# nglaze00/SCoNe_GCN

Hardware: NVIDIA B200
Metric: SCoNe train trajectories/sec (higher is better)
Workload: dtype f32

## Files before the change

### include/scone_b200.h

```cpp
#ifndef SCONE_B200_H
#define SCONE_B200_H

#include <stdint.h>

#ifdef __cplusplus
extern "C" {
#endif

#define SCONE_B200_VERSION 100
#define SCONE_MAX_DEGREE 128

typedef struct scone_complex scone_complex;
typedef struct scone_model scone_model;

enum { SCONE_MODEL_SCONE = 0, SCONE_MODEL_EBLI = 1, SCONE_MODEL_BUNCH = 2 };
enum { SCONE_ACT_TANH = 0, SCONE_ACT_LEAKY_RELU = 1, SCONE_ACT_RELU = 2 };

int scone_version(void);
const char* scone_last_error(void);

int scone_complex_create(int32_t n_nodes, int32_t n_edges, int32_t n_tris,
                         const int32_t* edge_nodes , const int8_t* edge_signs ,
                         const int32_t* tri_edges , const int8_t* tri_signs ,
                         int32_t model, scone_complex** out);
// ... 67 lines not shown
                              const float* flow_val, const int32_t* last_nodes, const int32_t* n_nbrs,
                              const int32_t* target_idx, const float* mask, int32_t* out_host , void* stream);
int scone_model_eval_host(scone_model* m, int32_t B, const int32_t* traj_ptr, const int32_t* flow_edge, const float* flow_val,
                          const int32_t* last_nodes, const int32_t* n_nbrs, const int32_t* target_idx, const float* mask,
                          int32_t* choice_out, int32_t* acc_out, float* nll_out, void* stream);
int scone_model_two_target_host(scone_model* m, int32_t B, const int32_t* true_idx, const int32_t* rand_idx, int32_t* out ,
                                void* stream);
int scone_model_read_grads(scone_model* m, float* out_host, void* stream);
int scone_model_read_grads_async(scone_model* m, float* out_pinned, void* stream);

int scone_model_adam_step(scone_model* m, int32_t step, float lr, float weight_decay, void* stream);

typedef struct scone_dp scone_dp;
int scone_dp_create(int32_t rank, int32_t world, int64_t n_floats, scone_dp** out);
int32_t scone_dp_handle_bytes(void);
int scone_dp_get_handle(scone_dp* dp, void* handle_out);
int scone_dp_open(scone_dp* dp, const void* handles_rank_major);
int scone_model_dp_adam_step(scone_model* m, scone_dp* dp, int32_t step, float lr, float wd, void* stream);
int scone_dp_status(scone_dp* dp, void* stream);
void scone_dp_destroy(scone_dp* dp);
int scone_model_plan_host(scone_model* m, int32_t B, const int32_t* traj_ptr, const int32_t* flow_edge, const float* flow_val,
                          const int32_t* last_nodes, void* stream);
int scone_model_plan_dev(scone_model* m, int32_t B, const int32_t* traj_ptr_dev, const int32_t* flow_edge_dev, const float* flow_val_dev,
                         const int32_t* last_nodes_dev, void* stream);
int scone_model_loss_grad_planned_host(scone_model* m, int32_t n, const int32_t* rows, const int32_t* target_idx, const float* mask,
                                       int32_t zero_first, void* stream);
int scone_model_loss_grad_planned_dev(scone_model* m, int32_t n, const int32_t* rows_dev, const int32_t* target_idx_dev, const float* mask_dev,
                                      int32_t zero_first, void* stream);
int scone_model_forward_planned_host(scone_model* m, int32_t n, const int32_t* rows, float* logprobs_out , void* stream);
int scone_model_check_overflow(scone_model* m, void* stream);
int scone_model_set_weights_keep_state(scone_model* m, const float* weights_host, void* stream);
int scone_model_fused_info(const scone_model* m, int32_t* out );
int scone_model_fused_read(scone_model* m, int32_t t, int32_t* hdr_out , uint32_t off, int32_t words, uint32_t* arena_out);
int scone_model_read_rows_done(scone_model* m, int64_t* out );

typedef struct scone_csr scone_csr;
typedef struct scone_bunch scone_bunch;
int scone_csr_create(int32_t rows, int32_t cols, const int32_t* rowptr , const int32_t* col, const float* val,
                     scone_csr** out);
int scone_csr_destroy(scone_csr* S);
int scone_bunch_create(const scone_csr* const* S7, int32_t n_nodes, int32_t n_edges, int32_t n_tris, int32_t max_degree,
                       const int32_t* nbrhoods , int32_t n_hidden, const int32_t* hidden,
                       int32_t micro_batch, scone_bunch** out);
int scone_bunch_destroy(scone_bunch* m);
int64_t scone_bunch_num_params(const scone_bunch* m);
float* scone_bunch_grads_dev(scone_bunch* m);
int scone_bunch_set_weights(scone_bunch* m, const float* weights_host, int32_t reset_adam);
int scone_bunch_get_weights(const scone_bunch* m, float* weights_host);
int scone_bunch_forward_host(scone_bunch* m, int32_t B, const int32_t* traj_ptr, const int32_t* flow_edge, const float* flow_val,
                             const int32_t* last_nodes, float* logprobs_out , void* stream);
int scone_bunch_loss_grad_host(scone_bunch* m, int32_t B, const int32_t* traj_ptr, const int32_t* flow_edge, const float* flow_val,
                               const int32_t* last_nodes, const int32_t* target_idx, const float* mask, int32_t zero_first,
                               void* stream);
int scone_bunch_read_grads(scone_bunch* m, float* out_host, void* stream);
int scone_bunch_adam_step(scone_bunch* m, int32_t step, float lr, float weight_decay, void* stream);

int scone_set_zero_fill(int32_t on);
int scone_get_zero_fill(void);

int scone_set_dense_kernel(int32_t which);
int scone_umma_status(void* stream);
int scone_set_dense_chunk(int32_t tiles);
int scone_get_dense_kernel(void);

int scone_profile_enable(int32_t on);
int scone_profile_reset(void);
// ... 10 lines not shown
```

### scone_gcn_b200/_lib.py

```python
import ctypes as C
import os

_HERE = os.path.dirname(os.path.abspath(__file__))
_LIB = None


class LibraryMissing(RuntimeError):
    pass


class SconeError(RuntimeError):
    pass


def library_path():
    return os.path.join(_HERE, 'libscone_b200.so')


_i32, _i64, _f32, _vp = C.c_int32, C.c_int64, C.c_float, C.c_void_p
DEFAULT_DENSE_KERNEL = 3

SIGNATURES = {
    'scone_version': (C.c_int, []),
    'scone_last_error': (C.c_char_p, []),
# ... 42 lines not shown
    'scone_model_set_pipeline': (C.c_int, [_vp, _i32]),
    'scone_model_get_pipeline': (C.c_int, [_vp]),
    'scone_model_set_weights': (C.c_int, [_vp, _vp]),
    'scone_model_get_weights': (C.c_int, [_vp, _vp]),
    'scone_model_weights_dev': (_vp, [_vp]),
    'scone_model_grads_dev': (_vp, [_vp]),
    'scone_model_forward_host': (C.c_int, [_vp, _i32, _vp, _vp, _vp, _vp, _vp, _vp]),
    'scone_model_forward_dev': (C.c_int, [_vp, _i32, _vp, _vp, _vp, _vp, _vp, _vp]),
    'scone_model_loss_grad_dev': (C.c_int, [_vp, _i32, _vp, _vp, _vp, _vp, _vp, _vp, _i32, _vp]),
    'scone_model_loss_grad_host': (C.c_int, [_vp, _i32, _vp, _vp, _vp, _vp, _vp, _vp, _i32, _vp]),
    'scone_accuracy_dev': (C.c_int, [_i32, _i32, _vp, _vp, _vp, _vp, _vp, _vp]),
    'scone_model_accuracy_host': (C.c_int, [_vp, _i32, _vp, _vp, _vp, _vp, _vp, _vp, _vp, _vp, _vp]),
    'scone_model_read_grads': (C.c_int, [_vp, _vp, _vp]),
    'scone_model_read_grads_async': (C.c_int, [_vp, _vp, _vp]),
    'scone_model_eval_host': (C.c_int, [_vp, _i32] + [_vp] * 10 + [_vp]),
    'scone_model_two_target_host': (C.c_int, [_vp, _i32, _vp, _vp, _vp, _vp]),
    'scone_model_adam_step': (C.c_int, [_vp, _i32, _f32, _f32, _vp]),
    'scone_dp_create': (C.c_int, [_i32, _i32, _i64, C.POINTER(_vp)]),
    'scone_dp_handle_bytes': (_i32, []),
    'scone_dp_get_handle': (C.c_int, [_vp, _vp]),
    'scone_dp_open': (C.c_int, [_vp, _vp]),
    'scone_model_dp_adam_step': (C.c_int, [_vp, _vp, _i32, _f32, _f32, _vp]),
    'scone_dp_status': (C.c_int, [_vp, _vp]),
    'scone_dp_destroy': (None, [_vp]),
    'scone_model_check_overflow': (C.c_int, [_vp, _vp]),
    'scone_model_plan_host': (C.c_int, [_vp, _i32, _vp, _vp, _vp, _vp, _vp]),
    'scone_model_plan_dev': (C.c_int, [_vp, _i32, _vp, _vp, _vp, _vp, _vp]),
    'scone_model_loss_grad_planned_host': (C.c_int, [_vp, _i32, _vp, _vp, _vp, _i32, _vp]),
    'scone_model_loss_grad_planned_dev': (C.c_int, [_vp, _i32, _vp, _vp, _vp, _i32, _vp]),
    'scone_model_forward_planned_host': (C.c_int, [_vp, _i32, _vp, _vp, _vp]),
    'scone_model_set_weights_keep_state': (C.c_int, [_vp, _vp, _vp]),
    'scone_model_fused_info': (C.c_int, [_vp, _vp]),
    'scone_model_fused_read': (C.c_int, [_vp, _i32, _vp, C.c_uint32, _i32, _vp]),
    'scone_model_read_rows_done': (C.c_int, [_vp, _vp]),
}


def lib():
    global _LIB
    if _LIB is not None:
        return _LIB
    path = library_path()
    if not os.path.exists(path):
        raise LibraryMissing(
            '%s not found: build it with `python __graft_entry__.py build` (or `make`). '
            'scone_gcn_b200 has no CPU fallback.' % path)
    L = C.CDLL(path)
    for name, (res, args) in SIGNATURES.items():
        f = getattr(L, name)
        f.restype, f.argtypes = res, args
    _LIB = L
    return L


def check(rc, what=''):
    if rc != 0:
        msg = lib().scone_last_error().decode('utf-8', 'replace')
        raise SconeError('%s failed (code %d): %s' % (what or 'scone call', rc, msg))


def ptr(a):
    if a is None:
        return None
    assert a.flags['C_CONTIGUOUS']
    return a.ctypes.data_as(C.c_void_p)

# ... 9 lines not shown
```

### scone_gcn_b200/csrc/fused.cuh

```cuda
#pragma once
#include "common.cuh"

constexpr int kFusedMaxL = 3;
constexpr int kFusedHdrW = 16;
constexpr int kFusedFlagOverflow = 1;
constexpr int kFusedFlagRetry = 2;

struct PlanArgs {
    const int32_t* traj_ptr;
    const int32_t* flow_edge;
    const float* flow_val;
    const int32_t* last_nodes;
    const int32_t* rank;
    const int32_t* nbrhoods;
    const int32_t* inc_ptr;
    const int2* inc_ent;
    const int32_t* mptr;
    const int2* ment;
    int N, D, E, L;
    int HS, hshift;
    const unsigned* cone_ptr;
    const uint32_t* cone_ent;
    int LV;
    int EC;
    int M;
    const unsigned long long* node_off;
    const unsigned* tb_rowptr;
    const int2* tb_ent;
    const unsigned* pair_ptr;
    const int2* tb_pairs;
    const int* pair_off;
    int* hdr;
    uint32_t* arena;
    unsigned long long* bump;
    unsigned long long arena_words;
    int* overflow;
    int tier;
    int n_work;
    int t0;
    const int* n_in;
    const int* in_list;
    int* n_retry;
    int* retry;
};

#ifdef __CUDACC__
template <int THREADS>
__device__ inline int fused_block_scan_excl(int* a, int n, int* s_warp) {
    const int tid = threadIdx.x, lane = tid & 31, warp = tid >> 5;
    const int per = (n + THREADS - 1) / THREADS;
    const int lo = min(n, tid * per), hi = min(n, lo + per);
    int sum = 0;
    for (int i = lo; i < hi; ++i) sum += a[i];
    int inc = sum;
#pragma unroll
    for (int o = 1; o < 32; o <<= 1) {
        const int v = __shfl_up_sync(0xffffffffu, inc, o);
        if (lane >= o) inc += v;
    }
    __syncthreads();
    if (lane == 31) s_warp[warp] = inc;
    __syncthreads();
    int base = 0, total = 0;
#pragma unroll
    for (int w = 0; w < THREADS / 32; ++w) {
        const int v = s_warp[w];
        if (w < warp) base += v;
        total += v;
    }
    int run = base + inc - sum;
    for (int i = lo; i < hi; ++i) {
        const int v = a[i];
        a[i] = run;
        run += v;
    }
    if (tid == 0) a[n] = total;
    __syncthreads();
    return total;
}
#endif

struct FusedState {
    int L = 0, C = 0;
    int64_t n_params = 0;
    int bound_cone = 0, bound_list = 0;
    unsigned* d_cone_ptr = nullptr;
    uint32_t* d_cone_ent = nullptr;
    unsigned long long cone_entries = 0;
    bool tb_rows = false;
    unsigned long long* d_node_off = nullptr;
    unsigned* d_tb_rowptr = nullptr;
    int2* d_tb_ent = nullptr;
    unsigned* d_pair_ptr = nullptr;
    int2* d_tb_pairs = nullptr;
    int* d_pair_off = nullptr;
    unsigned long long tb_entries = 0, tb_bytes = 0;
    int tbM0 = 0, tbLV0 = 0, tbM1 = 0, tbLV1 = 0, tbM = 0, tbLV = 0;
    size_t tb_smem0 = 0, tb_smem1 = 0, tb_smem = 0;
    bool tb_two_tiers = false, tb_mid_tier = false;
    int quantile_cone = 0;
    int HS = 0, LV = 0, EC = 0, hshift = 0;
    int HS0 = 0, LV0 = 0, EC0 = 0, hshift0 = 0;
    bool two_tiers = false;
    int flow_room = 0;
    size_t plan_smem0 = 0;
    unsigned long long worst_words = 0;
    int* d_retry = nullptr;
    size_t plan_smem = 0, traj_smem_small = 0, traj_smem_big = 0;
    int cap_rows = 0, big_rows = 0, grid_small = 0, grid_big = 0, chunk = 0;
    size_t scratch_stride = 0;
    unsigned long long arena_words = 0;
    int* d_hdr = nullptr;
    uint32_t* d_arena = nullptr;
    unsigned long long* d_bump = nullptr;
    float* d_partial = nullptr;
    float* d_scratch = nullptr;
    int* d_stats = nullptr;
    unsigned long long* d_rows_done = nullptr;
    uint32_t* d_sort = nullptr;
    void* d_sort_tmp = nullptr;
    size_t sort_tmp_bytes = 0;
    int sort_cap = 0;
    int* d_set_hdr = nullptr;
    uint32_t* d_set_arena = nullptr;
    unsigned long long* d_set_bump = nullptr;
    unsigned long long set_arena_words = 0;
    int set_cap = 0, set_n = 0;
};

int scone_table_build(const scone_complex* cx, FusedState* f, int L, bool* ok);
int scone_table_plan_launch(const FusedState* f, PlanArgs p, int b, int num_sms, cudaStream_t st, int phase = 2);
void scone_table_destroy(FusedState* f);
// ... 22 lines not shown
```

### scone_gcn_b200/csrc/scone_fused.cu

```cuda
#include <algorithm>
#include <cstdlib>
#include <cub/device/device_radix_sort.cuh>
#include "common.cuh"
#include "fused.cuh"

namespace {

#include "slab_common.cuh"

constexpr int kTrajThreads = 256;
constexpr int kFuMaxD = SCONE_MAX_DEGREE;
constexpr uint32_t kNoRow = 0xFFFFu;
constexpr uint32_t kFlaggedKey = 0xFFFFFFu;

template <int ACT>
__device__ __forceinline__ float fu_act(float z) {
    if (ACT == SCONE_ACT_TANH) return scone_tanh(z);
    if (ACT == SCONE_ACT_LEAKY_RELU) return z >= 0.f ? z : 0.01f * z;
    return fmaxf(z, 0.f);
}
template <int ACT>
__device__ __forceinline__ float fu_dact(float h) {
    if (ACT == SCONE_ACT_TANH) return 1.f - h * h;
    if (ACT == SCONE_ACT_LEAKY_RELU) return h >= 0.f ? 1.f : 0.01f;
// ... 1095 lines not shown
    f->cap_rows = C == 32 ? 192 : 384;
    f->big_rows = L * f->bound_list;
    f->traj_smem_small = C == 32 ? traj_smem_bytes<32>(cx->D, f->cap_rows) : traj_smem_bytes<16>(cx->D, f->cap_rows);
    f->traj_smem_big = C == 32 ? traj_smem_bytes<32>(cx->D, 0) : traj_smem_bytes<16>(cx->D, 0);
    if (f->traj_smem_small > 113 * 1024) {
        const size_t over = f->traj_smem_small - 113 * 1024;
        const int less = (int)((over + ldh * 4 - 1) / (ldh * 4));
        f->cap_rows = f->cap_rows > less + 32 ? f->cap_rows - less : 32;
        f->traj_smem_small = C == 32 ? traj_smem_bytes<32>(cx->D, f->cap_rows) : traj_smem_bytes<16>(cx->D, f->cap_rows);
    }
    f->grid_small = 2 * cx->num_sms;
    f->grid_big = f->big_rows > f->cap_rows ? 2 * cx->num_sms : 0;
    if (f->grid_big) {
        f->scratch_stride = (size_t)f->big_rows * ldh;
        SCONE_CUDA(cudaMalloc((void**)&f->d_scratch, (size_t)f->grid_big * f->scratch_stride * sizeof(float)));
    }
    SCONE_CUDA(cudaMalloc((void**)&f->d_partial, (size_t)(f->grid_small + f->grid_big) * (n_params + 2) * sizeof(float)));
    const unsigned long long bl = (unsigned long long)f->bound_list;
    unsigned long long worst = 3 * bl + 2 + (unsigned long long)(cx->D + 3) + 2ull * cx->D * cx->D + 16;
    for (int l = 2; l <= L; ++l)
        worst += 2 * (bl + 3) + 4 * bl * (unsigned long long)max_row;
    const unsigned long long budget_words = (1ull << 30) - 1024;
    const unsigned long long share_words = 16 * 1024;
    f->worst_words = worst;
    if (worst * (unsigned long long)mb <= budget_words) {
        f->chunk = mb;
        f->arena_words = worst * (unsigned long long)mb;
    } else {
        f->chunk = (int)std::min<unsigned long long>((unsigned long long)mb, std::max<unsigned long long>(1, budget_words / std::min(worst, share_words)));
        f->arena_words = std::min(budget_words, worst * (unsigned long long)f->chunk);
    }
    SCONE_CUDA(cudaMalloc((void**)&f->d_arena, f->arena_words * sizeof(uint32_t)));
    SCONE_CUDA(cudaMalloc((void**)&f->d_hdr, (size_t)f->chunk * kFusedHdrW * sizeof(int)));
    SCONE_CUDA(cudaMalloc((void**)&f->d_retry, 2 * (size_t)f->chunk * sizeof(int)));
    SCONE_CUDA(cudaMalloc((void**)&f->d_bump, 2 * sizeof(unsigned long long)));
    SCONE_CUDA(cudaMalloc((void**)&f->d_rows_done, 4 * sizeof(unsigned long long)));
    SCONE_CUDA(cudaMemset(f->d_rows_done, 0, 4 * sizeof(unsigned long long)));
    *out = f;
    return 0;
}

static int launch_plans(const scone_complex* cx, const FusedState* f, PlanArgs p, int b, cudaStream_t st) {
    if (f->tb_rows) return scone_table_plan_launch(f, p, b, cx->num_sms, st);
    p.tier = 0; p.n_work = b;
    p.HS = f->HS0; p.LV = f->LV0; p.EC = f->EC0; p.hshift = f->hshift0;
    int* retry = p.retry;
    if (!f->two_tiers) p.retry = nullptr;
    fused_plan_kernel<256><<<b, 256, f->plan_smem0, st>>>(p);
    SCONE_LAUNCHED();
    if (f->two_tiers) {
        p.tier = 1; p.HS = f->HS; p.LV = f->LV; p.EC = f->EC; p.hshift = f->hshift; p.n_in = p.n_retry; p.in_list = retry; p.retry = nullptr;
        fused_plan_kernel<1024><<<std::min(b, cx->num_sms), 1024, f->plan_smem, st>>>(p);
        SCONE_LAUNCHED();
    }
    return 0;
}

int scone_fused_begin(FusedState* f, cudaStream_t st) {
    SCONE_CUDA(cudaMemsetAsync(f->d_bump, 0, 2 * sizeof(unsigned long long), st));
    return 0;
}

static PlanArgs plan_args(const scone_complex* cx, FusedState* f, int off, const int32_t* traj_ptr, const int32_t* flow_edge,
                          const float* flow_val, const int32_t* last_nodes, int* overflow) {
    PlanArgs p{};
    p.traj_ptr = traj_ptr + off; p.flow_edge = flow_edge; p.flow_val = flow_val; p.last_nodes = last_nodes + off;
    p.rank = cx->d_rank; p.nbrhoods = cx->d_nbrhoods; p.inc_ptr = cx->d_inc_ptr; p.inc_ent = cx->d_inc_ent;
    p.mptr = cx->d_mptr; p.ment = cx->d_ment; p.cone_ptr = f->d_cone_ptr; p.cone_ent = f->d_cone_ent;
// ... 31 lines not shown
    t.hdr = f->d_hdr; t.arena = f->d_arena; t.rows = nullptr; t.W = W;
    for (int i = 0; i <= 3 * kFusedMaxL; ++i) t.w_off[i] = i <= 3 * f->L ? (int)w_off[i] : 0;
    t.L = f->L; t.b = b; t.D = cx->D; t.n_params = (int)f->n_params;
    t.logprobs = logprobs; t.target_idx = target_idx; t.mask = mask;
    t.partial = f->d_partial; t.scratch = f->d_scratch; t.scratch_stride = f->scratch_stride;
    t.cap_rows = f->cap_rows; t.big_rows = f->big_rows;
    t.rows_done = count_rows ? f->d_rows_done : nullptr;
    return run_traj(f, act, t, grad, st);
}

int scone_fused_run(const scone_complex* cx, FusedState* f, int act, int b, const int32_t* traj_ptr, const int32_t* flow_edge,
                    const float* flow_val, const int32_t* last_nodes, const float* W, const int64_t* w_off, float* logprobs,
                    const int32_t* target_idx, const float* mask, float* grad, int* overflow, bool count_rows, cudaStream_t st) {
    if (b <= 0) return 0;
    SCONE_REQUIRE(b <= f->chunk, "scone_fused_run: chunk of %d trajectories exceeds the planned %d", b, f->chunk);
    int rc = scone_fused_begin(f, st);
    if (!rc) rc = scone_fused_plan_part(cx, f, 0, b, traj_ptr, flow_edge, flow_val, last_nodes, overflow, st);
    if (!rc) rc = scone_fused_compute(cx, f, act, b, W, w_off, logprobs, target_idx, mask, grad, count_rows, st);
    return rc;
}

int scone_fused_plan_set(const scone_complex* cx, FusedState* f, int B, const int32_t* traj_ptr, const int32_t* flow_edge,
                         const float* flow_val, const int32_t* last_nodes, int* overflow, cudaStream_t st) {
    if (B > f->set_cap) {
        cudaFree(f->d_set_hdr);
        cudaFree(f->d_set_arena);
        f->d_set_hdr = nullptr;
        f->d_set_arena = nullptr;
        f->set_cap = 0;
        const unsigned long long budget_words = (1ull << 30) - 1024;
        f->set_arena_words = std::min(budget_words, f->worst_words * (unsigned long long)B);
        SCONE_CUDA(cudaMalloc((void**)&f->d_set_hdr, (size_t)B * kFusedHdrW * sizeof(int)));
        SCONE_CUDA(cudaMalloc((void**)&f->d_set_arena, f->set_arena_words * sizeof(uint32_t)));
        if (!f->d_set_bump) SCONE_CUDA(cudaMalloc((void**)&f->d_set_bump, 2 * sizeof(unsigned long long)));
        f->set_cap = B;
    }
    f->set_n = 0;
    SCONE_CUDA(cudaMemsetAsync(f->d_set_bump, 0, 2 * sizeof(unsigned long long), st));
    PlanArgs p{};
    p.flow_edge = flow_edge; p.flow_val = flow_val;
    p.rank = cx->d_rank; p.nbrhoods = cx->d_nbrhoods; p.inc_ptr = cx->d_inc_ptr; p.inc_ent = cx->d_inc_ent;
    p.mptr = cx->d_mptr; p.ment = cx->d_ment; p.cone_ptr = f->d_cone_ptr; p.cone_ent = f->d_cone_ent;
    p.N = cx->N; p.D = cx->D; p.E = cx->E; p.L = f->L;
    p.arena = f->d_set_arena; p.bump = f->d_set_bump; p.arena_words = f->set_arena_words; p.overflow = overflow;
    p.n_retry = reinterpret_cast<int*>(f->d_set_bump + 1); p.retry = f->d_retry;
    ScopedProf prof(SCONE_K_CONE, st);
    for (int off = 0; off < B; off += f->chunk) {
        const int b = std::min(f->chunk, B - off);
        SCONE_CUDA(cudaMemsetAsync(f->d_set_bump + 1, 0, sizeof(unsigned long long), st));
        p.traj_ptr = traj_ptr + off; p.last_nodes = last_nodes + off; p.hdr = f->d_set_hdr + (size_t)off * kFusedHdrW;
        const int rc = launch_plans(cx, f, p, b, st);
        if (rc) return rc;
    }
    f->set_n = B;
    return 0;
}

int scone_fused_run_planned(const scone_complex* cx, FusedState* f, int act, int n, const int32_t* rows_dev, const float* W, const int64_t* w_off,
                            float* logprobs, const int32_t* target_idx, const float* mask, float* grad, bool count_rows, cudaStream_t st) {
    if (n <= 0) return 0;
    SCONE_REQUIRE(f->set_n > 0, "scone_fused_run_planned: no planned set (call scone_model_plan_* first)");
    SCONE_REQUIRE(rows_dev != nullptr || n <= f->set_n, "scone_fused_run_planned: %d trajectories requested, the planned set holds %d", n, f->set_n);
    TrajArgs t;
    t.hdr = f->d_set_hdr; t.arena = f->d_set_arena; t.rows = rows_dev; t.W = W;
    for (int i = 0; i <= 3 * kFusedMaxL; ++i) t.w_off[i] = i <= 3 * f->L ? (int)w_off[i] : 0;
    t.L = f->L; t.b = n; t.D = cx->D; t.n_params = (int)f->n_params;
    t.logprobs = logprobs; t.target_idx = target_idx; t.mask = mask;
// ... 20 lines not shown
```

### scone_gcn_b200/csrc/scone_model.cu

```cuda
#include <algorithm>
#include <cstring>
#include "common.cuh"
#include "fused.cuh"

struct scone_model {
    const scone_complex* cx = nullptr;
    int32_t L = 0, mb = 0, act = 0, cmax = 0;
    std::vector<int32_t> hidden;
    std::vector<int64_t> w_off;
    int64_t n_params = 0;
    float *d_w = nullptr, *d_m = nullptr, *d_v = nullptr, *d_grad = nullptr;
    float* d_X = nullptr;
    std::vector<float*> d_H;
    std::vector<float*> d_G;
    std::vector<uint8_t*> d_occH;
    std::vector<uint8_t*> d_occG;
    cudaStream_t side = nullptr;
    cudaStream_t compute = nullptr;
    cudaEvent_t ev_fork = nullptr, ev_join = nullptr;
    cudaEvent_t ev_begin = nullptr;
    cudaStream_t copy = nullptr;
    cudaEvent_t ev_copy0 = nullptr, ev_part[8] = {nullptr, nullptr, nullptr, nullptr, nullptr, nullptr, nullptr, nullptr};
    cudaEvent_t ev_plan_done = nullptr;
    long long staging_epoch = 0, plan_done_epoch = -1;
// ... 1051 lines not shown
    cudaStream_t s = as_stream(st);
    if (m->d_overflow) SCONE_CUDA(cudaMemcpyAsync(&overflow, m->d_overflow, sizeof(int), cudaMemcpyDeviceToHost, s));
    SCONE_CUDA(cudaStreamSynchronize(s));
    if (overflow) {
        cudaMemset(m->d_overflow, 0, sizeof(int));
        m->cone_clean = false;
        scone_set_error("scone_model: a micro-batch exceeded a row-list capacity (%d rows per compact tensor, %d rows of the backward's A "
                        "buffer, 2048 cone edges per trajectory and layer); results since the last check are incomplete and Adam steps were "
                        "skipped — use a smaller micro-batch or another pipeline", m->row_cap, m->a_cap);
        return 4;
    }
    return 0;
}

extern "C" int scone_model_set_weights_keep_state(scone_model* m, const float* w, void* st) {
    SCONE_REQUIRE(m && w, "scone_model_set_weights_keep_state: NULL argument");
    SCONE_CUDA(cudaMemcpyAsync(m->d_w, w, m->n_params * sizeof(float), cudaMemcpyHostToDevice, as_stream(st)));
    return 0;
}

extern "C" int scone_model_fused_info(const scone_model* m, int32_t* out ) {
    SCONE_REQUIRE(m && out, "scone_model_fused_info: NULL argument");
    for (int i = 0; i < 16; ++i) out[i] = 0;
    if (!m->fused) return 0;
    const FusedState* f = m->fused;
    out[0] = 1; out[1] = f->bound_cone; out[2] = f->bound_list; out[3] = f->HS; out[4] = f->chunk; out[5] = f->cap_rows;
    out[6] = (int32_t)(f->plan_smem / 1024); out[7] = (int32_t)(f->traj_smem_small / 1024);
    out[8] = f->HS0; out[9] = f->LV0; out[10] = (int32_t)(f->plan_smem0 / 1024); out[11] = f->two_tiers ? 1 : 0;
    out[12] = f->tb_rows ? (int32_t)std::max<unsigned long long>(1, f->tb_bytes >> 20) : 0; out[13] = (int32_t)(f->arena_words >> 20);
    out[14] = (int32_t)std::min<unsigned long long>(f->cone_entries >> 10, 0x7fffffffull); out[15] = scone_fused_last_retries(m->fused);
    return 0;
}

extern "C" int scone_model_fused_read(scone_model* m, int32_t t, int32_t* hdr_out, uint32_t off, int32_t words, uint32_t* arena_out) {
    SCONE_REQUIRE(m && m->fused, "scone_model_fused_read: the model has no fused pipeline");
    SCONE_REQUIRE(t >= 0 && t < m->fused->chunk && (uint64_t)off + (uint64_t)(words > 0 ? words : 0) <= m->fused->arena_words,
                  "scone_model_fused_read: out of range");
    return scone_fused_read(m->fused, t, hdr_out, off, words, arena_out);
}

extern "C" int scone_model_read_rows_done(scone_model* m, int64_t* out ) {
    SCONE_REQUIRE(m && out, "scone_model_read_rows_done: NULL argument");
    out[0] = out[1] = 0;
    if (!m->fused) return 0;
    unsigned long long v[2];
    SCONE_CUDA(cudaMemcpy(v, m->fused->d_rows_done, sizeof(v), cudaMemcpyDeviceToHost));
    SCONE_CUDA(cudaMemset(m->fused->d_rows_done, 0, sizeof(v)));
    out[0] = (int64_t)v[0];
    out[1] = (int64_t)v[1];
    return 0;
}

extern "C" int scone_umma_status(void* st) { return scone_umma_check(as_stream(st)); }

extern "C" int scone_model_dp_adam_step(scone_model* m, scone_dp* dp, int32_t step, float lr, float wd, void* st) {
    SCONE_REQUIRE(m && dp && step >= 0, "scone_model_dp_adam_step: bad arguments");
    return scone_dp_allreduce_adam(dp, m->d_w, m->d_m, m->d_v, m->d_grad, m->n_params, m->d_overflow, step, lr, wd, as_stream(st));
}

extern "C" int scone_model_adam_step(scone_model* m, int32_t step, float lr, float wd, void* st) {
    SCONE_REQUIRE(m && step >= 0, "scone_model_adam_step: bad arguments");
    return scone_adam_launch(m->d_w, m->d_m, m->d_v, m->d_grad, m->n_params, step, lr, wd, st, m->d_overflow);
}
```

### scone_gcn_b200/csrc/scone_plan_table.cu

```cuda
#include <algorithm>
#include <cstdlib>
#include <vector>
#include "common.cuh"
#include "fused.cuh"

namespace {

constexpr int kTbThreads = 256;
constexpr int kTbHS = 32768;
constexpr int kTbLC = 16384;
constexpr uint32_t kEdgeMask = 0x3FFFFFFFu;
constexpr uint32_t kEmpty = 0xFFFFFFFFu;
constexpr uint32_t kNoRow = 0xFFFFu;
constexpr int kTbMaxD = SCONE_MAX_DEGREE;
constexpr int kTbBuckets = 1024;

__device__ __forceinline__ int align2(int x) { return (x + 1) & ~1; }

struct BuildArgs {
    const int32_t* nbrhoods;
    const int32_t* inc_ptr;
    const int2* inc_ent;
    const int32_t* mptr;
    const int2* ment;
    int N, D, L;
    int* stats;
    int* cnt_m;
    unsigned* cnt_e;
    int* cnt_p;
    const unsigned* cone_ptr;
    uint32_t* keys;
    int with_rows;
    const unsigned long long* node_off;
    unsigned* rowptr;
    int2* ent;
    const unsigned* pair_ptr;
    int2* pairs;
    int* pair_off;
};

__device__ __forceinline__ int find_sorted(const uint32_t* s, int m, uint32_t e) {
    int lo = 0, hi = m;
    while (lo < hi) {
        const int mid = (lo + hi) >> 1;
        if ((s[mid] & kEdgeMask) < e) lo = mid + 1;
        else hi = mid;
    }
    return lo < m && (s[lo] & kEdgeMask) == e ? lo : -1;
}

__global__ void __launch_bounds__(kTbThreads) table_build_kernel(const BuildArgs a) {
    extern __shared__ __align__(16) unsigned char sm[];
    uint32_t* hk = reinterpret_cast<uint32_t*>(sm);
    uint32_t* list = hk + kTbHS;
    __shared__ int s_ptr[kTbMaxD], s_off[kTbMaxD + 1];
    __shared__ int s_nlist, s_m, s_n1, s_ovf, s_nat[kFusedMaxL + 2], s_warp[kTbThreads / 32];
    __shared__ unsigned s_etot;
    const int tid = threadIdx.x, lane = tid & 31, ql = tid & 3;
    const unsigned qmask = 0xFu << (lane & ~3);
    const int node = blockIdx.x, D = a.D, L = a.L;
    const bool fill = a.keys != nullptr;
    for (int i = tid; i < kTbHS; i += kTbThreads) hk[i] = kEmpty;
// ... 62 lines not shown
    __syncthreads();
    int f0 = 0;
    for (int lv = L - 1; lv >= 0; --lv) {
        const int f1 = s_nat[lv + 1];
        if (!s_ovf)
            for (int i = f0 + (tid >> 2); i < f1; i += kTbThreads / 4) {
                const int e = (int)list[i];
                const int p1 = a.mptr[e + 1];
                for (int q = a.mptr[e] + ql; q < p1; q += 4) add((uint32_t)a.ment[q].x, lv);
            }
        __syncthreads();
        if (tid == 0) s_nat[lv] = min(s_nlist, kTbLC);
        __syncthreads();
        f0 = f1;
    }
    const int m = s_m;
    const bool bad = s_ovf != 0 || m > cap;
    if (!fill) {
        if (!bad) {
            unsigned c = 0;
            const int n1 = s_nlist;
            for (int i = tid >> 2; i < n1; i += kTbThreads / 4) {
                const int e = (int)list[i];
                const int p1 = a.mptr[e + 1];
                for (int q = a.mptr[e] + ql; q < p1; q += 4) c += level_of((uint32_t)a.ment[q].x) == 0 ? 2u : 1u;
            }
            if (c) atomicAdd(&s_etot, c);
        }
        __syncthreads();
        if (tid == 0) {
            a.cnt_m[node] = bad ? 0 : m;
            a.cnt_e[node] = bad ? 0u : s_etot;
            a.cnt_p[node] = total_pairs;
            if (bad) a.stats[2] = 1;
            else {
                atomicMax(&a.stats[0], m);
                atomicMax(&a.stats[1], s_n1);
                atomicMax(&a.stats[3], total_pairs);
                atomicAdd(&a.stats[4 + min(kTbBuckets - 1, m / 32)], 1);
            }
        }
        return;
    }
    if (bad) {
        if (tid == 0) a.stats[2] = 1;
        return;
    }
    __syncthreads();
    uint32_t* tmp = hk;
    for (int i = tid; i < m; i += kTbThreads) tmp[i] = kout[i];
    __syncthreads();
    uint32_t* sorted = list;
    for (int k = tid; k < m; k += kTbThreads) {
        const uint32_t v = tmp[k], e = v & kEdgeMask;
        int r = 0;
        for (int q = 0; q < m; ++q) r += (tmp[q] & kEdgeMask) < e ? 1 : 0;
        sorted[r] = v;
    }
    __syncthreads();
    for (int i = tid; i < m; i += kTbThreads) kout[i] = sorted[i];
    if (a.with_rows) {
        for (int i = tid; i < total_pairs; i += kTbThreads) {
            const int j = slot_of(i);
            const int2 es = a.inc_ent[s_ptr[j] + (i - s_off[j])];
            const int li = find_sorted(sorted, m, (uint32_t)es.x);
            a.pairs[a.pair_ptr[node] + i] = make_int2((int)((li >= 0 ? (uint32_t)li : kNoRow) | ((uint32_t)j << 16)), es.y);
// ... 361 lines not shown
    {
        const uint16_t* idxL = idx + (L - 1) * M;
        int* pdst = reinterpret_cast<int*>(a.arena + off_ro);
        int2* edst = reinterpret_cast<int2*>(a.arena + off_ro + align2(D + 1));
        for (int j = tid; j <= D; j += THREADS) pdst[j] = last_ok ? a.pair_off[(size_t)last * (D + 1) + j] : 0;
        for (int i = tid; i < total_pairs; i += THREADS) {
            const int2 pr = a.tb_pairs[pp0 + i];
            const uint32_t li = (uint32_t)pr.x & 0xFFFFu;
            const uint32_t r = li != kNoRow ? (uint32_t)idxL[li] : kNoRow;
            edst[i] = make_int2((int)(r | ((uint32_t)pr.x & 0xFFFF0000u)), pr.y);
        }
    }
    if (tid == 0) {
        hdr[0] = 0;
        for (int l = 1; l <= kFusedMaxL; ++l) hdr[l] = l <= L ? n_l[l] : 0;
        hdr[4] = (int)off_l1;
        for (int l = 2; l <= kFusedMaxL; ++l) {
            hdr[5 + (l - 2)] = (int)off_f[l];
            hdr[7 + (l - 2)] = (int)off_b[l];
        }
        hdr[9] = (int)off_ro;
        hdr[10] = total_pairs;
        hdr[11] = m;
        hdr[12] = tot_f[2];
        hdr[13] = fp1 - fp0;
        hdr[14] = tot_f[3];
        hdr[15] = min(tot_b[2], 0xFFFF) | (min(tot_b[3], 0xFFFF) << 16);
    }
}

template <int THREADS>
__global__ void __launch_bounds__(THREADS) table_plan_kernel(const PlanArgs a) {
    extern __shared__ __align__(16) unsigned char sm[];
    const int n_work = a.tier == 0 ? a.n_work : *a.n_in;
    for (int w = blockIdx.x; w < n_work; w += gridDim.x) {
        table_plan_trajectory<THREADS>(a, a.tier == 0 ? a.t0 + w : a.in_list[w], sm);
        __syncthreads();
    }
}

constexpr int kTier1Threads = 512;
constexpr size_t kMaxTablePlanSmem = 220 * 1024;

}

void scone_table_destroy(FusedState* f) {
    cudaFree(f->d_cone_ptr); cudaFree(f->d_cone_ent); cudaFree(f->d_node_off); cudaFree(f->d_tb_rowptr); cudaFree(f->d_tb_ent);
    cudaFree(f->d_pair_ptr); cudaFree(f->d_tb_pairs); cudaFree(f->d_pair_off);
    f->d_cone_ptr = nullptr; f->d_cone_ent = nullptr; f->d_node_off = nullptr; f->d_tb_rowptr = nullptr; f->d_tb_ent = nullptr;
    f->d_pair_ptr = nullptr; f->d_tb_pairs = nullptr; f->d_pair_off = nullptr;
    f->tb_rows = false;
}

int scone_table_build(const scone_complex* cx, FusedState* f, int L, bool* ok) {
    *ok = false;
    const int N = cx->N, D = cx->D;
    if (D > kTbMaxD || N < 1) return 0;
    const int n_stats = 4 + kTbBuckets;
    SCONE_CUDA(cudaMalloc((void**)&f->d_stats, n_stats * sizeof(int)));
    SCONE_CUDA(cudaMemset(f->d_stats, 0, n_stats * sizeof(int)));
    const size_t smem = (size_t)kTbHS * 4 + (size_t)kTbLC * 4;
    SCONE_CUDA(cudaFuncSetAttribute(table_build_kernel, cudaFuncAttributeMaxDynamicSharedMemorySize, (int)smem));
    int* d_cnt_m = nullptr;
    unsigned* d_cnt_e = nullptr;
    int* d_cnt_p = nullptr;
    SCONE_CUDA(cudaMalloc((void**)&d_cnt_m, (size_t)N * sizeof(int)));
    SCONE_CUDA(cudaMalloc((void**)&d_cnt_e, (size_t)N * sizeof(unsigned)));
    SCONE_CUDA(cudaMalloc((void**)&d_cnt_p, (size_t)N * sizeof(int)));
    BuildArgs a{};
    a.nbrhoods = cx->d_nbrhoods; a.inc_ptr = cx->d_inc_ptr; a.inc_ent = cx->d_inc_ent; a.mptr = cx->d_mptr; a.ment = cx->d_ment;
    a.N = N; a.D = D; a.L = L; a.stats = f->d_stats;
    a.cnt_m = d_cnt_m; a.cnt_e = d_cnt_e; a.cnt_p = d_cnt_p;
    table_build_kernel<<<N, kTbThreads, smem>>>(a);
    SCONE_LAUNCHED();
    std::vector<int> st(n_stats), cm((size_t)N), cp((size_t)N);
    std::vector<unsigned> ce((size_t)N);
    SCONE_CUDA(cudaMemcpy(st.data(), f->d_stats, n_stats * sizeof(int), cudaMemcpyDeviceToHost));
    SCONE_CUDA(cudaMemcpy(cm.data(), d_cnt_m, (size_t)N * sizeof(int), cudaMemcpyDeviceToHost));
    SCONE_CUDA(cudaMemcpy(ce.data(), d_cnt_e, (size_t)N * sizeof(unsigned), cudaMemcpyDeviceToHost));
    SCONE_CUDA(cudaMemcpy(cp.data(), d_cnt_p, (size_t)N * sizeof(int), cudaMemcpyDeviceToHost));
    cudaFree(d_cnt_m); cudaFree(d_cnt_e); cudaFree(d_cnt_p);
    std::vector<unsigned> cone_ptr((size_t)N + 1), pair_ptr((size_t)N + 1);
    std::vector<unsigned long long> node_off((size_t)N + 1);
    unsigned long long tm = 0, te = 0, tp = 0;
    for (int n = 0; n < N; ++n) {
        cone_ptr[n] = (unsigned)tm; node_off[n] = te; pair_ptr[n] = (unsigned)tp;
        tm += (unsigned long long)cm[n]; te += ce[n]; tp += (unsigned long long)cp[n];
    }
    if (st[2] || tm + (unsigned long long)N + 1 >= (1ull << 32) || tp >= (1ull << 32)) return 0;
    cone_ptr[N] = (unsigned)tm; node_off[N] = te; pair_ptr[N] = (unsigned)tp;
    f->cone_entries = tm;
    int quantile999 = 0;
    f->bound_cone = st[0] > 0 ? st[0] : 1;
    f->bound_list = st[1] > 0 ? st[1] : 1;
    {
        long long acc = 0, want = ((long long)N * 99 + 99) / 100;
        int q0 = 32 * kTbBuckets;
        for (int b = 0; b < kTbBuckets; ++b) {
            acc += st[4 + b];
            if (acc >= want) {
                q0 = 32 * (b + 1);
                break;
            }
        }
        f->quantile_cone = std::min(q0, f->bound_cone);
        acc = 0;
        want = ((long long)N * 999 + 999) / 1000;
        quantile999 = f->bound_cone;
        for (int b = 0; b < kTbBuckets; ++b) {
            acc += st[4 + b];
            if (acc >= want) {
                quantile999 = std::min(32 * (b + 1), f->bound_cone);
                break;
            }
        }
    }
    const unsigned long long bytes = te * 8 + (tm + (unsigned long long)N + 1) * 4 + tp * 8 + (unsigned long long)N * (D + 1) * 4 + ((unsigned long long)N + 1) * 16;
    bool want_rows = true;
    {
        const char* v = getenv("SCONE_FUSED_TABLE");
        if (v && *v == '0') want_rows = false;
        size_t free_b = 0, total_b = 0;
        SCONE_CUDA(cudaMemGetInfo(&free_b, &total_b));
        if (bytes > free_b / 3) want_rows = false;
        f->tbM = (f->bound_cone + 63) & ~63;
        f->tbLV = (f->bound_list + 63) & ~63;
        f->tb_smem = table_plan_smem(f->tbM, f->tbLV);
        if (f->tb_smem > kMaxTablePlanSmem || f->bound_cone >= 0xFFFF || f->bound_list >= 0xFFFF) want_rows = false;
    }
    SCONE_CUDA(cudaMalloc((void**)&f->d_cone_ptr, cone_ptr.size() * sizeof(unsigned)));
    SCONE_CUDA(cudaMalloc((void**)&f->d_cone_ent, (size_t)(tm ? tm : 1) * sizeof(uint32_t)));
    SCONE_CUDA(cudaMemcpy(f->d_cone_ptr, cone_ptr.data(), cone_ptr.size() * sizeof(unsigned), cudaMemcpyHostToDevice));
    a.cnt_m = nullptr; a.cnt_e = nullptr; a.cnt_p = nullptr;
    a.cone_ptr = f->d_cone_ptr; a.keys = f->d_cone_ent; a.with_rows = want_rows ? 1 : 0;
    if (want_rows) {
        SCONE_CUDA(cudaMalloc((void**)&f->d_node_off, node_off.size() * sizeof(unsigned long long)));
        SCONE_CUDA(cudaMalloc((void**)&f->d_tb_rowptr, (size_t)(tm + N + 1) * sizeof(unsigned)));
        SCONE_CUDA(cudaMalloc((void**)&f->d_tb_ent, (size_t)(te ? te : 1) * sizeof(int2)));
        SCONE_CUDA(cudaMalloc((void**)&f->d_pair_ptr, pair_ptr.size() * sizeof(unsigned)));
        SCONE_CUDA(cudaMalloc((void**)&f->d_tb_pairs, (size_t)(tp ? tp : 1) * sizeof(int2)));
        SCONE_CUDA(cudaMalloc((void**)&f->d_pair_off, (size_t)N * (D + 1) * sizeof(int)));
        SCONE_CUDA(cudaMemcpy(f->d_node_off, node_off.data(), node_off.size() * sizeof(unsigned long long), cudaMemcpyHostToDevice));
        SCONE_CUDA(cudaMemcpy(f->d_pair_ptr, pair_ptr.data(), pair_ptr.size() * sizeof(unsigned), cudaMemcpyHostToDevice));
        a.node_off = f->d_node_off; a.rowptr = f->d_tb_rowptr; a.ent = f->d_tb_ent;
        a.pair_ptr = f->d_pair_ptr; a.pairs = f->d_tb_pairs; a.pair_off = f->d_pair_off;
    }
    table_build_kernel<<<N, kTbThreads, smem>>>(a);
    SCONE_LAUNCHED();
    SCONE_CUDA(cudaDeviceSynchronize());
    SCONE_CUDA(cudaMemcpy(st.data(), f->d_stats, 4 * sizeof(int), cudaMemcpyDeviceToHost));
    if (st[2] == 1) return 0;
    if (st[2] == 2) {
        want_rows = false;
        SCONE_CUDA(cudaMemset(f->d_stats + 2, 0, sizeof(int)));
        cudaFree(f->d_node_off); cudaFree(f->d_tb_rowptr); cudaFree(f->d_tb_ent); cudaFree(f->d_pair_ptr); cudaFree(f->d_tb_pairs); cudaFree(f->d_pair_off);
        f->d_node_off = nullptr; f->d_tb_rowptr = nullptr; f->d_tb_ent = nullptr; f->d_pair_ptr = nullptr; f->d_tb_pairs = nullptr; f->d_pair_off = nullptr;
    }
    f->tb_rows = want_rows;
    if (want_rows) {
        f->tb_entries = te;
        f->tb_bytes = bytes;
        auto env_int = [](const char* name, int dflt) {
            const char* v = getenv(name);
            return v && *v ? atoi(v) : dflt;
        };
        f->tbM0 = std::min(f->tbM, (env_int("SCONE_TABLE_M0", f->quantile_cone) + 63) & ~63);
        f->tbLV0 = std::min(f->tbLV, (env_int("SCONE_TABLE_LV0", 192) + 63) & ~63);
        f->tb_two_tiers = f->tbM0 < f->tbM || f->tbLV0 < f->tbLV;
        f->tb_smem0 = table_plan_smem(f->tbM0, f->tbLV0);
        f->tbM1 = std::min(f->tbM, (env_int("SCONE_TABLE_M1", std::max(quantile999, 2 * f->tbM0)) + 63) & ~63);
        f->tbLV1 = std::min(f->tbLV, (env_int("SCONE_TABLE_LV1", 512) + 63) & ~63);
        f->tb_smem1 = table_plan_smem(f->tbM1, f->tbLV1);
        f->tb_mid_tier = f->tb_two_tiers && (f->tbM1 > f->tbM0 || f->tbLV1 > f->tbLV0) && 2 * f->tb_smem1 <= f->tb_smem;
        SCONE_CUDA(cudaFuncSetAttribute(table_plan_kernel<64>, cudaFuncAttributeMaxDynamicSharedMemorySize, (int)kMaxTablePlanSmem));
        SCONE_CUDA(cudaFuncSetAttribute(table_plan_kernel<128>, cudaFuncAttributeMaxDynamicSharedMemorySize, (int)kMaxTablePlanSmem));
        SCONE_CUDA(cudaFuncSetAttribute(table_plan_kernel<256>, cudaFuncAttributeMaxDynamicSharedMemorySize, (int)kMaxTablePlanSmem));
        SCONE_CUDA(cudaFuncSetAttribute(table_plan_kernel<kTier1Threads>, cudaFuncAttributeMaxDynamicSharedMemorySize, (int)kMaxTablePlanSmem));
    }
    *ok = true;
    return 0;
}

int scone_table_plan_launch(const FusedState* f, PlanArgs p, int b, int num_sms, cudaStream_t st, int phase) {
    const int f_chunk = f->chunk;
    p.cone_ptr = f->d_cone_ptr; p.cone_ent = f->d_cone_ent; p.node_off = f->d_node_off; p.tb_rowptr = f->d_tb_rowptr; p.tb_ent = f->d_tb_ent;
    p.pair_ptr = f->d_pair_ptr; p.tb_pairs = f->d_tb_pairs; p.pair_off = f->d_pair_off;
    p.tier = 0; p.n_work = b;
    p.M = f->tbM0; p.LV = f->tbLV0;
    int* list0 = p.retry;
    int* list1 = p.retry + f_chunk;
    int* cnt0 = p.n_retry;
    int* cnt1 = p.n_retry + 1;
    p.retry = f->tb_two_tiers ? list0 : nullptr;
    p.n_retry = cnt0;
    if (phase != 1) {
        static const int t0 = [] { const char* v = getenv("SCONE_TABLE_T0"); return v && *v ? atoi(v) : 128; }();
        if (t0 == 64) table_plan_kernel<64><<<b, 64, f->tb_smem0, st>>>(p);
        else if (t0 == 256) table_plan_kernel<256><<<b, 256, f->tb_smem0, st>>>(p);
        else table_plan_kernel<128><<<b, 128, f->tb_smem0, st>>>(p);
        SCONE_LAUNCHED();
    }
    if (!f->tb_two_tiers || phase == 0) return 0;
    const int* n_in = cnt0;
    const int* in_list = list0;
    if (f->tb_mid_tier) {
        p.tier = 1; p.M = f->tbM1; p.LV = f->tbLV1; p.n_in = n_in; p.in_list = in_list; p.retry = list1; p.n_retry = cnt1;
        const int per_sm = std::max(1, std::min(8, (int)((size_t)220 * 1024 / (f->tb_smem1 + 1024))));
        table_plan_kernel<256><<<std::min(b, per_sm * num_sms), 256, f->tb_smem1, st>>>(p);
        SCONE_LAUNCHED();
        n_in = cnt1;
        in_list = list1;
    }
    p.tier = 2; p.M = f->tbM; p.LV = f->tbLV; p.n_in = n_in; p.in_list = in_list; p.retry = nullptr; p.n_retry = cnt0;
    const int per_sm = std::max(1, std::min(4, (int)((size_t)220 * 1024 / (f->tb_smem + 1024))));
    table_plan_kernel<512><<<std::min(b, per_sm * num_sms), 512, f->tb_smem, st>>>(p);
    SCONE_LAUNCHED();
    return 0;
}
```

Before: 7.431 million.

## Route trajectories to plan tiers up front and overlap tier kernels with PDL

Cone sizes per node are classified into tiers at table build time, and a small routing kernel sends each trajectory straight to its tier list by its last node. The heavy tier-2 kernel is launched first, and the mid and tier-0 kernels follow as programmatic dependent launches so they can overlap with it. This replaces the serial retry cascade, where every trajectory first tried tier 0 and overflowed down through the tiers. A fallback tier-2 pass runs only if a node's level count can exceed its tier limit, at the cost of an extra routing launch and more complex scheduling.

```diff
diff --git a/include/scone_b200.h b/include/scone_b200.h
--- a/include/scone_b200.h
+++ b/include/scone_b200.h
@@ -123,6 +123,7 @@
 int scone_model_set_weights_keep_state(scone_model* m, const float* weights_host, void* stream);
 int scone_model_fused_info(const scone_model* m, int32_t* out );
 int scone_model_fused_read(scone_model* m, int32_t t, int32_t* hdr_out , uint32_t off, int32_t words, uint32_t* arena_out);
+int scone_model_plan_tiers(const scone_model* m, int32_t* params , uint8_t* tiers);
 int scone_model_read_rows_done(scone_model* m, int64_t* out );
 
 typedef struct scone_csr scone_csr;
diff --git a/scone_gcn_b200/_lib.py b/scone_gcn_b200/_lib.py
--- a/scone_gcn_b200/_lib.py
+++ b/scone_gcn_b200/_lib.py
@@ -98,6 +98,7 @@
     'scone_model_set_weights_keep_state': (C.c_int, [_vp, _vp, _vp]),
     'scone_model_fused_info': (C.c_int, [_vp, _vp]),
     'scone_model_fused_read': (C.c_int, [_vp, _i32, _vp, C.c_uint32, _i32, _vp]),
+    'scone_model_plan_tiers': (C.c_int, [_vp, _vp, _vp]),
     'scone_model_read_rows_done': (C.c_int, [_vp, _vp]),
 }
 
diff --git a/scone_gcn_b200/csrc/fused.cuh b/scone_gcn_b200/csrc/fused.cuh
--- a/scone_gcn_b200/csrc/fused.cuh
+++ b/scone_gcn_b200/csrc/fused.cuh
@@ -42,6 +42,7 @@
     const int* in_list;
     int* n_retry;
     int* retry;
+    const uint8_t* node_tier;
 };
 
 #ifdef __CUDACC__
@@ -98,6 +99,9 @@
     int tbM0 = 0, tbLV0 = 0, tbM1 = 0, tbLV1 = 0, tbM = 0, tbLV = 0;
     size_t tb_smem0 = 0, tb_smem1 = 0, tb_smem = 0;
     bool tb_two_tiers = false, tb_mid_tier = false;
+    uint8_t* d_tier = nullptr;
+    int tb_tier_nodes[3] = {0, 0, 0};
+    bool tb_tier_retry = false;
     int quantile_cone = 0;
     int HS = 0, LV = 0, EC = 0, hshift = 0;
     int HS0 = 0, LV0 = 0, EC0 = 0, hshift0 = 0;
diff --git a/scone_gcn_b200/csrc/scone_fused.cu b/scone_gcn_b200/csrc/scone_fused.cu
--- a/scone_gcn_b200/csrc/scone_fused.cu
+++ b/scone_gcn_b200/csrc/scone_fused.cu
@@ -1151,8 +1151,8 @@
     }
     SCONE_CUDA(cudaMalloc((void**)&f->d_arena, f->arena_words * sizeof(uint32_t)));
     SCONE_CUDA(cudaMalloc((void**)&f->d_hdr, (size_t)f->chunk * kFusedHdrW * sizeof(int)));
-    SCONE_CUDA(cudaMalloc((void**)&f->d_retry, 2 * (size_t)f->chunk * sizeof(int)));
-    SCONE_CUDA(cudaMalloc((void**)&f->d_bump, 2 * sizeof(unsigned long long)));
+    SCONE_CUDA(cudaMalloc((void**)&f->d_retry, 3 * (size_t)f->chunk * sizeof(int)));
+    SCONE_CUDA(cudaMalloc((void**)&f->d_bump, 3 * sizeof(unsigned long long)));
     SCONE_CUDA(cudaMalloc((void**)&f->d_rows_done, 4 * sizeof(unsigned long long)));
     SCONE_CUDA(cudaMemset(f->d_rows_done, 0, 4 * sizeof(unsigned long long)));
     *out = f;
@@ -1250,7 +1250,7 @@
         f->set_arena_words = std::min(budget_words, f->worst_words * (unsigned long long)B);
         SCONE_CUDA(cudaMalloc((void**)&f->d_set_hdr, (size_t)B * kFusedHdrW * sizeof(int)));
         SCONE_CUDA(cudaMalloc((void**)&f->d_set_arena, f->set_arena_words * sizeof(uint32_t)));
-        if (!f->d_set_bump) SCONE_CUDA(cudaMalloc((void**)&f->d_set_bump, 2 * sizeof(unsigned long long)));
+        if (!f->d_set_bump) SCONE_CUDA(cudaMalloc((void**)&f->d_set_bump, 3 * sizeof(unsigned long long)));
         f->set_cap = B;
     }
     f->set_n = 0;
diff --git a/scone_gcn_b200/csrc/scone_model.cu b/scone_gcn_b200/csrc/scone_model.cu
--- a/scone_gcn_b200/csrc/scone_model.cu
+++ b/scone_gcn_b200/csrc/scone_model.cu
@@ -1107,6 +1107,17 @@
     return 0;
 }
 
+extern "C" int scone_model_plan_tiers(const scone_model* m, int32_t* params, uint8_t* tiers) {
+    SCONE_REQUIRE(m && params, "scone_model_plan_tiers: NULL argument");
+    for (int i = 0; i < 8; ++i) params[i] = 0;
+    const FusedState* f = m->fused;
+    if (!f || !f->d_tier) return 0;
+    params[0] = 1; params[1] = f->tbM0; params[2] = f->tbLV0; params[3] = f->tbM1; params[4] = f->tbLV1; params[5] = f->tbM;
+    params[6] = f->tbLV; params[7] = f->tb_mid_tier ? 1 : 0;
+    if (tiers) SCONE_CUDA(cudaMemcpy(tiers, f->d_tier, (size_t)m->cx->N, cudaMemcpyDeviceToHost));
+    return 0;
+}
+
 extern "C" int scone_model_fused_read(scone_model* m, int32_t t, int32_t* hdr_out, uint32_t off, int32_t words, uint32_t* arena_out) {
     SCONE_REQUIRE(m && m->fused, "scone_model_fused_read: the model has no fused pipeline");
     SCONE_REQUIRE(t >= 0 && t < m->fused->chunk && (uint64_t)off + (uint64_t)(words > 0 ? words : 0) <= m->fused->arena_words,
diff --git a/scone_gcn_b200/csrc/scone_plan_table.cu b/scone_gcn_b200/csrc/scone_plan_table.cu
--- a/scone_gcn_b200/csrc/scone_plan_table.cu
+++ b/scone_gcn_b200/csrc/scone_plan_table.cu
@@ -1,5 +1,6 @@
 #include <algorithm>
 #include <cstdlib>
+#include <cstring>
 #include <vector>
 #include "common.cuh"
 #include "fused.cuh"
@@ -28,6 +29,7 @@
     int* cnt_m;
     unsigned* cnt_e;
     int* cnt_p;
+    int* cnt_n1;
     const unsigned* cone_ptr;
     uint32_t* keys;
     int with_rows;
@@ -156,6 +158,7 @@
             a.cnt_m[node] = bad ? 0 : m;
             a.cnt_e[node] = bad ? 0u : s_etot;
             a.cnt_p[node] = total_pairs;
+            a.cnt_n1[node] = bad ? 0 : s_n1;
             if (bad) a.stats[2] = 1;
             else {
                 atomicMax(&a.stats[0], m);
@@ -583,11 +586,51 @@
 template <int THREADS>
 __global__ void __launch_bounds__(THREADS) table_plan_kernel(const PlanArgs a) {
     extern __shared__ __align__(16) unsigned char sm[];
+    asm volatile("griddepcontrol.launch_dependents;");
     const int n_work = a.tier == 0 ? a.n_work : *a.n_in;
     for (int w = blockIdx.x; w < n_work; w += gridDim.x) {
-        table_plan_trajectory<THREADS>(a, a.tier == 0 ? a.t0 + w : a.in_list[w], sm);
+        const int t = a.tier == 0 ? a.t0 + w : a.in_list[w];
+        if (a.node_tier != nullptr) {
+            const int last = a.last_nodes[t];
+            if (last >= 0 && last < a.N && a.node_tier[last] != 0) continue;
+        }
+        table_plan_trajectory<THREADS>(a, t, sm);
         __syncthreads();
     }
+    if (blockIdx.x == gridDim.x - 1) asm volatile("griddepcontrol.wait;" ::: "memory");
+}
+
+__global__ void table_route_kernel(const int32_t* last_nodes, int t0, int b, int N, const uint8_t* node_tier, int* list1, int* list2,
+                                   int* cnt) {
+    const int w = blockIdx.x * blockDim.x + threadIdx.x;
+    if (w >= b) return;
+    const int t = t0 + w;
+    const int last = last_nodes[t];
+    const int k = last >= 0 && last < N ? node_tier[last] : 0;
+    if (k == 1) list1[atomicAdd(&cnt[0], 1)] = t;
+    else if (k == 2) list2[atomicAdd(&cnt[1], 1)] = t;
+}
+
+int env_per_sm(const char* name) {
+    const char* v = getenv(name);
+    return v && *v ? atoi(v) : 0;
+}
+
+template <typename Kernel>
+int launch_dependent(Kernel kern, int grid, int threads, size_t smem, cudaStream_t st, const PlanArgs& p) {
+    cudaLaunchAttribute attr[1];
+    attr[0].id = cudaLaunchAttributeProgrammaticStreamSerialization;
+    attr[0].val.programmaticStreamSerializationAllowed = 1;
+    cudaLaunchConfig_t cfg = {};
+    cfg.gridDim = dim3((unsigned)grid);
+    cfg.blockDim = dim3((unsigned)threads);
+    cfg.dynamicSmemBytes = smem;
+    cfg.stream = st;
+    cfg.attrs = attr;
+    cfg.numAttrs = 1;
+    SCONE_CUDA(cudaLaunchKernelEx(&cfg, kern, p));
+    SCONE_LAUNCHED();
+    return 0;
 }
 
 constexpr int kTier1Threads = 512;
@@ -597,7 +640,8 @@
 
 void scone_table_destroy(FusedState* f) {
     cudaFree(f->d_cone_ptr); cudaFree(f->d_cone_ent); cudaFree(f->d_node_off); cudaFree(f->d_tb_rowptr); cudaFree(f->d_tb_ent);
-    cudaFree(f->d_pair_ptr); cudaFree(f->d_tb_pairs); cudaFree(f->d_pair_off);
+    cudaFree(f->d_pair_ptr); cudaFree(f->d_tb_pairs); cudaFree(f->d_pair_off); cudaFree(f->d_tier);
+    f->d_tier = nullptr;
     f->d_cone_ptr = nullptr; f->d_cone_ent = nullptr; f->d_node_off = nullptr; f->d_tb_rowptr = nullptr; f->d_tb_ent = nullptr;
     f->d_pair_ptr = nullptr; f->d_tb_pairs = nullptr; f->d_pair_off = nullptr;
     f->tb_rows = false;
@@ -615,22 +659,25 @@
     int* d_cnt_m = nullptr;
     unsigned* d_cnt_e = nullptr;
     int* d_cnt_p = nullptr;
+    int* d_cnt_n1 = nullptr;
     SCONE_CUDA(cudaMalloc((void**)&d_cnt_m, (size_t)N * sizeof(int)));
     SCONE_CUDA(cudaMalloc((void**)&d_cnt_e, (size_t)N * sizeof(unsigned)));
     SCONE_CUDA(cudaMalloc((void**)&d_cnt_p, (size_t)N * sizeof(int)));
+    SCONE_CUDA(cudaMalloc((void**)&d_cnt_n1, (size_t)N * sizeof(int)));
     BuildArgs a{};
     a.nbrhoods = cx->d_nbrhoods; a.inc_ptr = cx->d_inc_ptr; a.inc_ent = cx->d_inc_ent; a.mptr = cx->d_mptr; a.ment = cx->d_ment;
     a.N = N; a.D = D; a.L = L; a.stats = f->d_stats;
-    a.cnt_m = d_cnt_m; a.cnt_e = d_cnt_e; a.cnt_p = d_cnt_p;
+    a.cnt_m = d_cnt_m; a.cnt_e = d_cnt_e; a.cnt_p = d_cnt_p; a.cnt_n1 = d_cnt_n1;
     table_build_kernel<<<N, kTbThreads, smem>>>(a);
     SCONE_LAUNCHED();
-    std::vector<int> st(n_stats), cm((size_t)N), cp((size_t)N);
+    std::vector<int> st(n_stats), cm((size_t)N), cp((size_t)N), cn1((size_t)N);
     std::vector<unsigned> ce((size_t)N);
     SCONE_CUDA(cudaMemcpy(st.data(), f->d_stats, n_stats * sizeof(int), cudaMemcpyDeviceToHost));
     SCONE_CUDA(cudaMemcpy(cm.data(), d_cnt_m, (size_t)N * sizeof(int), cudaMemcpyDeviceToHost));
     SCONE_CUDA(cudaMemcpy(ce.data(), d_cnt_e, (size_t)N * sizeof(unsigned), cudaMemcpyDeviceToHost));
     SCONE_CUDA(cudaMemcpy(cp.data(), d_cnt_p, (size_t)N * sizeof(int), cudaMemcpyDeviceToHost));
-    cudaFree(d_cnt_m); cudaFree(d_cnt_e); cudaFree(d_cnt_p);
+    SCONE_CUDA(cudaMemcpy(cn1.data(), d_cnt_n1, (size_t)N * sizeof(int), cudaMemcpyDeviceToHost));
+    cudaFree(d_cnt_m); cudaFree(d_cnt_e); cudaFree(d_cnt_p); cudaFree(d_cnt_n1);
     std::vector<unsigned> cone_ptr((size_t)N + 1), pair_ptr((size_t)N + 1);
     std::vector<unsigned long long> node_off((size_t)N + 1);
     unsigned long long tm = 0, te = 0, tp = 0;
@@ -682,7 +729,7 @@
     SCONE_CUDA(cudaMalloc((void**)&f->d_cone_ptr, cone_ptr.size() * sizeof(unsigned)));
     SCONE_CUDA(cudaMalloc((void**)&f->d_cone_ent, (size_t)(tm ? tm : 1) * sizeof(uint32_t)));
     SCONE_CUDA(cudaMemcpy(f->d_cone_ptr, cone_ptr.data(), cone_ptr.size() * sizeof(unsigned), cudaMemcpyHostToDevice));
-    a.cnt_m = nullptr; a.cnt_e = nullptr; a.cnt_p = nullptr;
+    a.cnt_m = nullptr; a.cnt_e = nullptr; a.cnt_p = nullptr; a.cnt_n1 = nullptr;
     a.cone_ptr = f->d_cone_ptr; a.keys = f->d_cone_ent; a.with_rows = want_rows ? 1 : 0;
     if (want_rows) {
         SCONE_CUDA(cudaMalloc((void**)&f->d_node_off, node_off.size() * sizeof(unsigned long long)));
@@ -727,6 +774,17 @@
         SCONE_CUDA(cudaFuncSetAttribute(table_plan_kernel<128>, cudaFuncAttributeMaxDynamicSharedMemorySize, (int)kMaxTablePlanSmem));
         SCONE_CUDA(cudaFuncSetAttribute(table_plan_kernel<256>, cudaFuncAttributeMaxDynamicSharedMemorySize, (int)kMaxTablePlanSmem));
         SCONE_CUDA(cudaFuncSetAttribute(table_plan_kernel<kTier1Threads>, cudaFuncAttributeMaxDynamicSharedMemorySize, (int)kMaxTablePlanSmem));
+        std::vector<uint8_t> tier((size_t)N);
+        for (int n = 0; n < N; ++n) {
+            int k = 2;
+            if (cm[n] <= f->tbM0) k = 0;
+            else if (f->tb_mid_tier && cm[n] <= f->tbM1) k = 1;
+            if ((k == 0 && cn1[n] > f->tbLV0) || (k == 1 && cn1[n] > f->tbLV1)) f->tb_tier_retry = true;
+            tier[n] = (uint8_t)k;
+            ++f->tb_tier_nodes[k];
+        }
+        SCONE_CUDA(cudaMalloc((void**)&f->d_tier, (size_t)N));
+        SCONE_CUDA(cudaMemcpy(f->d_tier, tier.data(), (size_t)N, cudaMemcpyHostToDevice));
     }
     *ok = true;
     return 0;
@@ -740,15 +798,45 @@
     p.M = f->tbM0; p.LV = f->tbLV0;
     int* list0 = p.retry;
     int* list1 = p.retry + f_chunk;
+    int* list2 = p.retry + 2 * f_chunk;
     int* cnt0 = p.n_retry;
     int* cnt1 = p.n_retry + 1;
+    int* cnt_route = p.n_retry + 2;
+    static const int t0 = [] { const char* v = getenv("SCONE_TABLE_T0"); return v && *v ? atoi(v) : 128; }();
+    auto (*tier0_kernel) = t0 == 64 ? table_plan_kernel<64> : (t0 == 256 ? table_plan_kernel<256> : table_plan_kernel<128>);
+    const int tier0_threads = t0 == 64 || t0 == 256 ? t0 : 128;
+    const char* sched = getenv("SCONE_PLAN_SCHEDULE");
+    const bool routed = f->tb_two_tiers && f->d_tier != nullptr && !(sched && strcmp(sched, "serial") == 0);
+    if (routed) {
+        if (phase != 1 && b > 0) {
+            SCONE_CUDA(cudaMemsetAsync(cnt_route, 0, 2 * sizeof(int), st));
+            table_route_kernel<<<(b + 255) / 256, 256, 0, st>>>(p.last_nodes, p.t0, b, p.N, f->d_tier, list1, list2, cnt_route);
+            SCONE_LAUNCHED();
+            const int per_sm_env[2] = {env_per_sm("SCONE_PLAN_TIER1_CTAS"), env_per_sm("SCONE_PLAN_TIER2_CTAS")};
+            const int per_sm1 = per_sm_env[0] > 0 ? per_sm_env[0] : std::max(1, std::min(8, (int)((size_t)220 * 1024 / (f->tb_smem1 + 1024))));
+            const int per_sm2 = per_sm_env[1] > 0 ? per_sm_env[1] : std::max(1, std::min(4, (int)((size_t)220 * 1024 / (f->tb_smem + 1024))));
+            PlanArgs h = p;
+            h.retry = nullptr;
+            h.tier = 2; h.M = f->tbM; h.LV = f->tbLV; h.n_in = cnt_route + 1; h.in_list = list2;
+            table_plan_kernel<kTier1Threads><<<std::min(b, per_sm2 * num_sms), kTier1Threads, f->tb_smem, st>>>(h);
+            SCONE_LAUNCHED();
+            if (f->tb_mid_tier) {
+                h.tier = 1; h.M = f->tbM1; h.LV = f->tbLV1; h.n_in = cnt_route; h.in_list = list1; h.retry = list0; h.n_retry = cnt0;
+                if (launch_dependent(table_plan_kernel<256>, std::min(b, per_sm1 * num_sms), 256, f->tb_smem1, st, h)) return 1;
+            }
+            p.retry = list0; p.n_retry = cnt0; p.node_tier = f->d_tier;
+            if (launch_dependent(tier0_kernel, b, tier0_threads, f->tb_smem0, st, p)) return 1;
+        }
+        if (phase == 0 || !f->tb_tier_retry) return 0;
+        p.tier = 2; p.M = f->tbM; p.LV = f->tbLV; p.n_in = cnt0; p.in_list = list0; p.retry = nullptr; p.node_tier = nullptr;
+        table_plan_kernel<kTier1Threads><<<std::min(b, num_sms), kTier1Threads, f->tb_smem, st>>>(p);
+        SCONE_LAUNCHED();
+        return 0;
+    }
     p.retry = f->tb_two_tiers ? list0 : nullptr;
     p.n_retry = cnt0;
     if (phase != 1) {
-        static const int t0 = [] { const char* v = getenv("SCONE_TABLE_T0"); return v && *v ? atoi(v) : 128; }();
-        if (t0 == 64) table_plan_kernel<64><<<b, 64, f->tb_smem0, st>>>(p);
-        else if (t0 == 256) table_plan_kernel<256><<<b, 256, f->tb_smem0, st>>>(p);
-        else table_plan_kernel<128><<<b, 128, f->tb_smem0, st>>>(p);
+        tier0_kernel<<<b, tier0_threads, f->tb_smem0, st>>>(p);
         SCONE_LAUNCHED();
     }
     if (!f->tb_two_tiers || phase == 0) return 0;
```

Result: faster. 7.566 million (median of 6 runs) (+1.8%).
